# congliuUvA/Clifford-Group-Equivariant-Simplicial-Message-Passing-Networks

Hardware: AMD Instinct MI355X
Metric: simplicial edges/sec (fwd+bwd) on Cl(3,0) 8-ch multivectors; % HBM roofline (higher is better)
Workload: dtype f32; 1 GPU; S1: EGCL layer fwd+bwd, Cl(1, 1, 1), 8 channels, 10000 nodes, 100000 edges/GPU x 1 GPU, aggr=mean, edge_attr 6ch, node_attr 3ch; aggregation=float atomics, launch=hip-graph replay

## Files before the change

clifford-group-equivariant-simplicial-message-passing-networks_amd/csrc/cemlp_cl.hpp:

```cpp
#pragma once
#include "cemlp_lane.hpp"

namespace csmpn {

constexpr int kClWaves = 4;
constexpr int kClSliceCap = 512;
constexpr int kClParStride = 36;

#define CL_LDS_ORDER() do { asm volatile("" ::: "memory"); __builtin_amdgcn_wave_barrier(); asm volatile("" ::: "memory"); } while (0)

struct ClStamp {
#ifdef CSMPN_STAMPS
    static constexpr int kSlots = 24;
    unsigned long long t0, acc[kSlots];
    CSMPN_DEV explicit ClStamp(int) {
#pragma unroll
        for (int i = 0; i < kSlots; ++i) acc[i] = 0;
        t0 = __builtin_amdgcn_s_memtime();
    }
    CSMPN_DEV void operator()(int id) {
        __builtin_amdgcn_sched_barrier(0);
        const unsigned long long t1 = __builtin_amdgcn_s_memtime();
        acc[id] += t1 - t0;
        t0 = t1;
// ... 48 lines not shown
            "v_fmac_f32_dpp %0, %8, %16 row_ror:%20 row_mask:0xf bank_mask:0xf\n\t"
            "v_fmac_f32_dpp %1, %9, %17 row_ror:%20 row_mask:0xf bank_mask:0xf\n\t"
            "v_fmac_f32_dpp %2, %10, %17 row_ror:%20 row_mask:0xf bank_mask:0xf\n\t"
            "v_fmac_f32_dpp %3, %11, %17 row_ror:%20 row_mask:0xf bank_mask:0xf\n\t"
            "v_fmac_f32_dpp %4, %12, %18 row_ror:%20 row_mask:0xf bank_mask:0xf\n\t"
            "v_fmac_f32_dpp %5, %13, %18 row_ror:%20 row_mask:0xf bank_mask:0xf\n\t"
            "v_fmac_f32_dpp %6, %14, %18 row_ror:%20 row_mask:0xf bank_mask:0xf\n\t"
            "v_fmac_f32_dpp %7, %15, %19 row_ror:%20 row_mask:0xf bank_mask:0xf"
            : "+v"(acc[0]), "+v"(acc[1]), "+v"(acc[2]), "+v"(acc[3]), "+v"(acc[4]), "+v"(acc[5]), "+v"(acc[6]), "+v"(acc[7])
            : "v"(x[0]), "v"(x[1]), "v"(x[2]), "v"(x[3]), "v"(x[4]), "v"(x[5]), "v"(x[6]), "v"(x[7]),
              "v"(w.x), "v"(w.y), "v"(w.z), "v"(w.w), "n"(ROT));
    }
}

template <int NK>
CSMPN_DEV void cl_pin(f4 (&w)[NK]) {
    if constexpr (NK == 8) asm volatile("" : "+v"(w[0]), "+v"(w[1]), "+v"(w[2]), "+v"(w[3]), "+v"(w[4]), "+v"(w[5]), "+v"(w[6]), "+v"(w[7]));
    else if constexpr (NK == 4) asm volatile("" : "+v"(w[0]), "+v"(w[1]), "+v"(w[2]), "+v"(w[3]));
    else if constexpr (NK == 2) asm volatile("" : "+v"(w[0]), "+v"(w[1]));
    else static_assert(NK == 1 || NK == 2 || NK == 4 || NK == 8, "batch size");
}
template <int C, int NROT, int TOFF, int BATCH = 4>
CSMPN_DEV void cl_mix(float (&acc)[8], const float (&x)[8], const float* ldsw) {
    static_assert(NROT % BATCH == 0, "whole batches");
#ifdef CL_X_NOMIX
    cl_fmac8<0>(acc, x, ld4(ldsw + TOFF));
    return;
#endif
    constexpr int NB = NROT / BATCH;
    f4 w[BATCH];
#pragma unroll
    for (int i = 0; i < BATCH; ++i) w[i] = ld4(ldsw + (TOFF + 4 * C * i));
    cl_pin<BATCH>(w);
    static_for<0, NB>([&](auto b) {
        f4 wn[BATCH];
        if constexpr (b + 1 < NB) {
#pragma unroll
            for (int i = 0; i < BATCH; ++i) wn[i] = ld4(ldsw + (TOFF + 4 * C * (BATCH * (b + 1) + i)));
        }
        static_for<0, BATCH>([&](auto i) { cl_fmac8<ClMap<C>::ROTL * (BATCH * b + i)>(acc, x, w[i]); });
        if constexpr (b + 1 < NB) {
            cl_pin<BATCH>(wn);
#pragma unroll
            for (int i = 0; i < BATCH; ++i) w[i] = wn[i];
        }
    });
}

constexpr int cl_pow2_ge(int w) { int p = 1; while (p < w) p <<= 1; return p; }

template <int C, int MODE, int NA, int K, bool BWD>
struct ClTab {
    static constexpr int NSEG = MODE == MODE_EDGE ? 1 : (MODE == MODE_NODE ? 2 : 0);
    static_assert(MODE == MODE_EDGE || MODE == MODE_NODE, "edge or node program");
    static constexpr int NP = K > 0 ? 1 : NSEG + (NA > 0 ? 1 : 0);
    static constexpr int width(int p) { return (K > 0 || p < NSEG) ? C : NA; }
    static constexpr int period(int p) { return (K > 0 || p < NSEG) ? C : cl_pow2_ge(NA); }
    static constexpr int coff(int p) { return C * p; }
    static constexpr int I = K > 0 ? C : NSEG * C + NA;
    static_assert(NA <= C, "attribute segment wider than the layer");
    static constexpr int W1(int p) { int o = 0; for (int q = 0; q < p; ++q) o += 4 * C * period(q); return o; }
    static constexpr int WR = W1(NP), WL = WR + 4 * C * C;
    static constexpr int fwd_end = WL + 4 * C * C;
    static constexpr int W1T(int p) { return fwd_end + 4 * C * C * p; }
    static constexpr int WRT = W1T(NP), WLT = WRT + 4 * C * C;
    static constexpr int par = BWD ? WLT + 4 * C * C : fwd_end;
    static constexpr int total = par + C * kClParStride;
    static constexpr int n_entries = par / 4;
};

template <int C>
CSMPN_DEV size_t cl_state_off(long row, int c) {
    constexpr int RPT = 64 / C;
    return (size_t)(row / RPT) * 512 + 4 * ((int)(row % RPT) * C + c);
}
struct ClFwd {
    float y[8], gate[4], R[8], invden[4], s[8];
    float qs, nl, invMn;
};

CSMPN_DEV float cl_smooth_abs_sqrt(float q) { return sqrt_pos(sqrt_pos(__builtin_fmaf(q, q, kSmooth))); }

template <class ALG, int C, class TB, bool BWD>
__device__ void cl_stage_block(const DevBlock& B, float* base, int tid, int dir) {
    constexpr int G = ALG::G, P = ALG::P, NE = TB::n_entries, NIT = (NE + 64 * kClWaves - 1) / (64 * kClWaves);
    static_assert(G == 4, "the weight of one (o, c) pair is one 16-byte vector of 4 grades");
    const float *pW1 = B.W1, *pWR = B.WR, *pWL = B.WL;
    const float* src[NIT];
#pragma unroll
    for (int it = 0; it < NIT; ++it) {
        const int e = tid + it * 64 * kClWaves;
        src[it] = nullptr;
        static_for<0, TB::NP>([&](auto p) {
            constexpr int e0 = TB::W1(p) / 4, PER = TB::period(p), n = PER * C;
            if (e >= e0 && e < e0 + n) {
                const int k = (e - e0) / C, o = (e - e0) % C, cs = (o + dir * k) & (PER - 1);
                if (cs < TB::width(p)) src[it] = pW1 + ((o * TB::I + TB::coff(p) + cs) * G);
            }
        });
        if (e >= TB::WR / 4 && e < TB::fwd_end / 4) {
            const int f = e - TB::WR / 4, which = f / (C * C), k = (f % (C * C)) / C, o = f % C, cs = (o + dir * k) & (C - 1);
            src[it] = (which == 0 ? pWR : pWL) + ((o * C + cs) * G);
        }
        if constexpr (BWD) {
            static_for<0, TB::NP>([&](auto p) {
                constexpr int e0 = TB::W1T(p) / 4, PER = TB::period(p);
                if (e >= e0 && e < e0 + C * C) {
                    const int k = (e - e0) / C, c = (e - e0) % C, o = (c + dir * k) & (C - 1), cs = c & (PER - 1);
                    if (cs < TB::width(p)) src[it] = pW1 + ((o * TB::I + TB::coff(p) + cs) * G);
                }
            });
            if (e >= TB::WRT / 4 && e < TB::par / 4) {
                const int f = e - TB::WRT / 4, which = f / (C * C), k = (f % (C * C)) / C, c = f % C, o = (c + dir * k) & (C - 1);
                src[it] = (which == 0 ? pWR : pWL) + ((o * C + c) * G);
            }
        }
    }
    f4 v[NIT];
#pragma unroll
    for (int it = 0; it < NIT; ++it) v[it] = src[it] ? ld4(src[it]) : f4{0.f, 0.f, 0.f, 0.f};
    constexpr int NPAR = C * kClParStride, NITP = (NPAR + 64 * kClWaves - 1) / (64 * kClWaves);
    static_assert(16 + P <= kClParStride, "parameter stride");
    const float *pb1 = B.b1, *pbL = B.bL, *pla = B.la, *psa = B.sa, *psb = B.sb, *pan = B.an, *pw = B.w;
    const bool has_b1 = B.has_b1 != 0;
    const float* ps[NITP];
    bool sig[NITP];
#pragma unroll
    for (int it = 0; it < NITP; ++it) {
        const int e = tid + it * 64 * kClWaves;
        ps[it] = nullptr;
        sig[it] = false;
        if (e < NPAR) {
            const int ch = e / kClParStride, s = e % kClParStride;
            if (s == 0) { if (has_b1) ps[it] = pb1 + ch; }
            else if (s == 1) ps[it] = pbL + ch;
            else if (s == 2) ps[it] = pla + ch;
            else if (s >= 4 && s < 8) ps[it] = psa + ch * G + (s - 4);
            else if (s >= 8 && s < 12) ps[it] = psb + ch * G + (s - 8);
            else if (s >= 12 && s < 16) { ps[it] = pan + ch * G + (s - 12); sig[it] = true; }
            else if (s >= 16 && s < 16 + P) ps[it] = pw + ch * P + (s - 16);
        }
    }
    float pv[NITP];
#pragma unroll
    for (int it = 0; it < NITP; ++it) pv[it] = ps[it] ? *ps[it] : 0.f;
#pragma unroll
    for (int it = 0; it < NIT; ++it) {
        const int e = tid + it * 64 * kClWaves;
        if (e < NE) st4(base + 4 * e, v[it]);
    }
#pragma unroll
    for (int it = 0; it < NITP; ++it) {
        const int e = tid + it * 64 * kClWaves;
        if (sig[it]) pv[it] = sigmoidf(pv[it]);
        if (e < NPAR) base[TB::par + e] = pv[it];
    }
}

template <class ALG>
CSMPN_DEV void cl_weighted_gp(float (&out)[8], const float (&z)[8], const float (&r)[8], const float* wp) {
    constexpr int P = ALG::P;
    f4 wv[(P + 3) / 4];
#pragma unroll
    for (int q = 0; q < (P + 3) / 4; ++q) wv[q] = ld4(wp + 4 * q);
    static_for<0, P>([&](auto p) {
        constexpr int gi = ALG::t.path_g[p][0], gj = ALG::t.path_g[p][1], gk = ALG::t.path_g[p][2];
        constexpr int i0 = ALG::gstart(gi), ni = ALG::gsize(gi);
        constexpr int j0 = ALG::gstart(gj), nj = ALG::gsize(gj);
        constexpr int k0 = ALG::gstart(gk), nk = ALG::gsize(gk);
        const float w = wv[p / 4][p % 4];
        float tmp[nj];
#pragma unroll
        for (int t = 0; t < nj; ++t) tmp[t] = 0.f;
        static_for<0, ni>([&](auto ii) {
            static_for<0, nk>([&](auto kk) {
                constexpr int i = i0 + ii, k = k0 + kk;
                constexpr int j = ALG::t.out[i][k];
                if constexpr (j >= j0 && j < j0 + nj) {
                    constexpr float sg = float(ALG::t.sign[i][k]);
                    tmp[j - j0] += (sg * z[i]) * r[k];
                }
            });
        });
#pragma unroll
        for (int t = 0; t < nj; ++t) out[j0 + t] = __builtin_fmaf(w, tmp[t], out[j0 + t]);
    });
}

template <class ALG, int C, class TB, int BATCH>
CSMPN_DEV void cl_block_tail(const float* ldsw, const float* ldsp, ClFwd& S, float (&out)[8], ClStamp& stamp, int sid, bool have_s = false) {
    constexpr int D = ALG::D, G = ALG::G;
    static_assert(D == 8 && G == 4, "Cl(3,0)-shaped algebra");
    const f4 p0 = ld4(ldsp + TB::par);
    const f4 sa = ld4(ldsp + (TB::par + 4)), sb = ld4(ldsp + (TB::par + 8));
    S.y[0] += p0.x;
    float z[D];
    static_for<0, G>([&](auto g) {
        constexpr int d0 = ALG::gstart(g), nd = ALG::gsize(g);
        float u;
        if constexpr (g == 0) {
            u = S.y[0];
        } else {
            u = 0.f;
            static_for<0, nd>([&](auto t) {
                constexpr int d = d0 + decltype(t)::value;
                u += qsf<ALG, d> * S.y[d] * S.y[d];
            });
        }
        S.gate[g] = sigmoidf(__builtin_fmaf(sa[int(g)], u, sb[int(g)]));
#pragma unroll
        for (int t = 0; t < nd; ++t) z[d0 + t] = S.gate[g] * S.y[d0 + t];
    });
    stamp(sid);
    float L[D];
#pragma unroll
    for (int d = 0; d < D; ++d) { S.R[d] = 0.f; L[d] = 0.f; }
    cl_mix<C, C, TB::WR, BATCH>(S.R, z, ldsw);
    if (have_s) {
        const f4 sg = ld4(ldsp + (TB::par + 12));
        static_for<0, G>([&](auto g) {
            constexpr int d0 = ALG::gstart(g), nd = ALG::gsize(g);
            float qq = 0.f;
            static_for<0, nd>([&](auto t) {
                constexpr int d = d0 + decltype(t)::value;
                qq += qsf<ALG, d> * S.R[d] * S.R[d];
            });
            const float m = __builtin_fmaf(sg[int(g)], cl_smooth_abs_sqrt(qq) - 1.0f, 1.0f);
            S.invden[g] = fast_rcp(m + kEps);
        });
        float qs = 0.f;
        static_for<0, D>([&](auto dd) {
            constexpr int d = decltype(dd)::value;
            qs += qsf<ALG, d> * S.s[d] * S.s[d];
        });
        S.qs = qs;
        S.nl = cl_smooth_abs_sqrt(qs);
        S.invMn = fast_rcp(__builtin_fmaf(cl_chan_sum<C>(S.nl), 1.0f / float(C), kEps));
        return;
    }
    cl_mix<C, C, TB::WL, BATCH>(L, z, ldsw);
// ... 197 lines not shown
    stamp(sid + 5);
    const f4 sa = ld4(ldsp + (TB::par + 4));
    static_for<0, G>([&](auto g) {
        constexpr int d0 = ALG::gstart(g), nd = ALG::gsize(g);
        float ggate = 0.f;
#pragma unroll
        for (int t = 0; t < nd; ++t) ggate = __builtin_fmaf(gz[d0 + t], S.y[d0 + t], ggate);
        const float gpre = ggate * S.gate[g] * (1.0f - S.gate[g]);
        float u;
        if constexpr (g == 0) {
            u = S.y[0];
        } else {
            u = 0.f;
            static_for<0, nd>([&](auto t) {
                constexpr int d = d0 + decltype(t)::value;
                u += qsf<ALG, d> * S.y[d] * S.y[d];
            });
        }
        sm.template add<RM::i_sa + 2 * g>(gpre * u);
        sm.template add<RM::i_sa + 2 * g + 1>(gpre);
        const float gu = gpre * sa[int(g)];
        static_for<0, nd>([&](auto t) {
            constexpr int d = d0 + decltype(t)::value;
            float v = gz[d] * S.gate[g];
            if constexpr (g == 0) v += gu;
            else v = __builtin_fmaf(gu * (2.0f * qsf<ALG, d>), S.y[d], v);
            gy[d] = v;
        });
    });
    sm.template add<RM::i_b1>(gy[0]);
    stamp(sid + 6);
}

CSMPN_DEV void cl_ld8(float (&x)[8], const float* p) {
    const f4 a = ld4(p), b = ld4(p + 4);
    x[0] = a.x; x[1] = a.y; x[2] = a.z; x[3] = a.w; x[4] = b.x; x[5] = b.y; x[6] = b.z; x[7] = b.w;
}
CSMPN_DEV void cl_st8(float* p, const float (&x)[8]) {
    st4(p, f4{x[0], x[1], x[2], x[3]});
    st4(p + 4, f4{x[4], x[5], x[6], x[7]});
}
#ifdef CL_X_NOOUT
#define CL_GST8(gp, lp, x) cl_st8(lp, x)
#else
#define CL_GST8(gp, lp, x) cl_st8(gp, x)
#endif

template <int C, int ROWLEN, bool SUB>
CSMPN_DEV void cl_scatter(const float* sc, int t_add, int t_sub, float* table, int lane) {
    using MP = ClMap<C>;
    constexpr int RPW = MP::RPW, SS = ROWLEN + 4, NC = ROWLEN / 64;
    static_assert(ROWLEN % 64 == 0, "whole columns");
    static_for<0, NC>([&](auto cc) {
        const int colx = 64 * cc + lane;
        const float* col = sc + colx;
        auto flush = [&](int target, float a) {
#ifndef CL_X_NOOUT
            if (target >= 0) atomicAdd(table + (size_t)target * ROWLEN + colx, a);
#else
            if (target == -12345) atomicAdd(table + (size_t)target * ROWLEN + colx, a);
#endif
        };
        float val[RPW];
#pragma unroll
        for (int i = 0; i < RPW; ++i) val[i] = col[i * SS];
        float acc = 0.f;
        int cur = __builtin_amdgcn_readlane(t_add, MP::lane_of_row(0));
        static_for<0, RPW>([&](auto rr) {
            const int t = __builtin_amdgcn_readlane(t_add, MP::lane_of_row(rr));
            if (t != cur) {
                flush(cur, acc);
                cur = t;
                acc = 0.f;
            }
            acc += val[rr];
        });
        flush(cur, acc);
        if constexpr (SUB) {
            static_for<0, RPW>([&](auto rr) { flush(__builtin_amdgcn_readlane(t_sub, MP::lane_of_row(rr)), -val[rr]); });
        }
    });
}

template <int C, int MODE>
struct ClTile {
    long row, lrow;
    bool valid;
    int i_dst, i_src, i_perm;
    float scale;
    template <int NA>
    CSMPN_DEV void load(const RowIO& io, long tile, int r) {
        row = tile * ClMap<C>::RPW + r;
        valid = row < io.rows;
        lrow = valid ? row : 0;
        i_dst = i_src = i_perm = 0;
        scale = 1.0f;
        if constexpr (MODE == MODE_EDGE) {
            i_dst = io.seg[0].ia[lrow];
            i_src = io.seg[0].ib[lrow];
            if constexpr (NA > 0) i_perm = io.seg[1].ia[lrow];
        }
        if constexpr (MODE == MODE_NODE) {
            if (io.seg[1].deg) { const int dg = io.seg[1].deg[lrow]; scale = 1.0f / float(dg > 1 ? dg : 1); }
        }
    }
};

template <class ALG, int C, int MODE, int NA>
struct ClRaw {
    static constexpr int NSEG = MODE == MODE_EDGE ? 2 : 2;
    f4 v[2 * (NSEG + (NA > 0 ? 1 : 0))];
    template <class TB>
    CSMPN_DEV void issue(const RowIO& io, const ClTile<C, MODE>& T, int c) {
        constexpr int D = ALG::D, ROW = C * D;
        const float *p0, *p1, *p2 = nullptr;
        if constexpr (MODE == MODE_EDGE) {
            p0 = io.seg[0].a + (size_t)T.i_dst * ROW + c * D;
            p1 = io.seg[0].b + (size_t)T.i_src * ROW + c * D;
            if constexpr (NA > 0) {
                const int ca = c & (TB::period(1) - 1);
                p2 = io.seg[1].a + (size_t)T.i_perm * (NA * D) + (ca < NA ? ca : NA - 1) * D;
            }
        } else {
            p0 = io.seg[0].a + (size_t)T.lrow * ROW + c * D;
            p1 = io.seg[1].a + (size_t)T.lrow * ROW + c * D;
            if constexpr (NA > 0) {
                const int ca = c & (TB::period(2) - 1);
                p2 = io.seg[2].a + (size_t)T.lrow * (NA * D) + (ca < NA ? ca : NA - 1) * D;
            }
        }
        v[0] = ld4(p0); v[1] = ld4(p0 + 4);
        v[2] = ld4(p1); v[3] = ld4(p1 + 4);
        if constexpr (NA > 0) { v[4] = ld4(p2); v[5] = ld4(p2 + 4); }
    }
    CSMPN_DEV void pin() {
        if constexpr (NA > 0) asm volatile("" : "+v"(v[0]), "+v"(v[1]), "+v"(v[2]), "+v"(v[3]), "+v"(v[4]), "+v"(v[5]));
        else asm volatile("" : "+v"(v[0]), "+v"(v[1]), "+v"(v[2]), "+v"(v[3]));
    }
    template <class TB>
    CSMPN_DEV void finish(float (&x)[TB::NP][8], const ClTile<C, MODE>& T) const {
        auto unpack = [&](float (&t)[8], const f4& a, const f4& b) {
            t[0] = a.x; t[1] = a.y; t[2] = a.z; t[3] = a.w; t[4] = b.x; t[5] = b.y; t[6] = b.z; t[7] = b.w;
        };
        if constexpr (MODE == MODE_EDGE) {
            const f4 a = v[0] - v[2], b = v[1] - v[3];
            unpack(x[0], a, b);
            if constexpr (NA > 0) unpack(x[1], v[4], v[5]);
        } else {
            unpack(x[0], v[0], v[1]);
            unpack(x[1], v[2] * T.scale, v[3] * T.scale);
            if constexpr (NA > 0) unpack(x[2], v[4], v[5]);
        }
    }
};

template <int C>
CSMPN_DEV int cl_probe_dir(int c) {
    const int probe = cl_dpp_i<0x120 + ClMap<C>::ROTL>(c);
    return (((probe - c) & (C - 1)) == 1) ? 1 : -1;
}

template <class ALG, int C, int MODE, int NBLK, int NA>
__global__ void __launch_bounds__(64 * kClWaves, 4) cemlp_cl_fwd_kernel(const DevCemlp C_arg, const RowIO io_arg) {
    CSMPN_KERNEL_ARGS(Cd);
    using MP = ClMap<C>;
    using T0 = ClTab<C, MODE, NA, 0, false>;
    using T1 = ClTab<C, MODE, NA, 1, false>;
    constexpr int D = ALG::D, ROW = C * D, RPW = MP::RPW, SS = ROW + 4;
    static_assert(NBLK == 1 || NBLK == 2, "one or two blocks");
    constexpr int tab_floats = T0::total + (NBLK > 1 ? T1::total : 0);
    constexpr int kBatch = 4;
    extern __shared__ __attribute__((aligned(16))) float smem[];
    float* lds = smem;
    const int wave = threadIdx.x >> 6, lane = threadIdx.x & 63;
    const int c = MP::chan(lane), r = MP::row(lane);
    float* sc = lds + tab_floats + wave * (RPW * SS);
    ClStamp stamp(0);
    const float* ldsw0 = lds + 4 * c;
    const float* ldsp0 = lds + kClParStride * c;
    const float* ldsw1 = ldsw0 + T0::total;
    const float* ldsp1 = ldsp0 + T0::total;

    const long ntiles = (io.rows + RPW - 1) / RPW;
    const long tstride = (long)gridDim.x * kClWaves;
    const bool save_s = NBLK > 1 && io.save_state != 0 && io.save != nullptr;
    const long tile0 = (long)blockIdx.x * kClWaves + wave;
    ClTile<C, MODE> T, Tn;
    T.template load<NA>(io, tile0, r);
    ClRaw<ALG, C, MODE, NA> raw;
    raw.template issue<T0>(io, T, c);
    Tn.template load<NA>(io, tile0 + tstride, r);
    {
        const int dir = cl_probe_dir<C>(c);
        cl_stage_block<ALG, C, T0, false>(Cd.b[0], lds, threadIdx.x, dir);
        if constexpr (NBLK > 1) cl_stage_block<ALG, C, T1, false>(Cd.b[1], lds + T0::total, threadIdx.x, dir);
    }
    __syncthreads();
    stamp(0);
    for (long tile = tile0; tile < ntiles; tile += tstride) {
        raw.pin();
        stamp(1);
        float out[D], in1[D];
        {
            float x[T0::NP][D];
            raw.template finish<T0>(x, T);
            ClFwd S;
#pragma unroll
            for (int d = 0; d < D; ++d) S.y[d] = 0.f;
            static_for<0, T0::NP>([&](auto p) { cl_mix<C, T0::period(p), T0::W1(p), kBatch>(S.y, x[p], ldsw0); });
            stamp(2);
            cl_block_tail<ALG, C, T0, kBatch>(ldsw0, ldsp0, S, out, stamp, 3);
            if (save_s && T.valid) {
                float* ps_ = io.save + state_region<ROW, ROW>(io.rows, 0, 0) + cl_state_off<C>(T.row, c);
                __builtin_nontemporal_store(f4{S.s[0], S.s[1], S.s[2], S.s[3]}, reinterpret_cast<f4*>(ps_));
                __builtin_nontemporal_store(f4{S.s[4], S.s[5], S.s[6], S.s[7]}, reinterpret_cast<f4*>(ps_ + 256));
            }
        }
        if constexpr (NBLK > 1) {
#pragma unroll
            for (int d = 0; d < D; ++d) in1[d] = out[d];
            ClFwd S;
#pragma unroll
            for (int d = 0; d < D; ++d) S.y[d] = 0.f;
            cl_mix<C, C, T1::W1(0), kBatch>(S.y, in1, ldsw1);
            stamp(8);
            cl_block_tail<ALG, C, T1, kBatch>(ldsw1, ldsp1, S, out, stamp, 9);
            if (save_s && T.valid) {
                float* ps_ = io.save + state_region<ROW, ROW>(io.rows, 0, 1) + cl_state_off<C>(T.row, c);
                __builtin_nontemporal_store(f4{S.s[0], S.s[1], S.s[2], S.s[3]}, reinterpret_cast<f4*>(ps_));
                __builtin_nontemporal_store(f4{S.s[4], S.s[5], S.s[6], S.s[7]}, reinterpret_cast<f4*>(ps_ + 256));
            }
        }
        const ClTile<C, MODE> Tc = T;
        T = Tn;
        raw.template issue<T0>(io, T, c);
        Tn.template load<NA>(io, tile + 2 * tstride, r);
        if constexpr (NBLK > 1) {
            if (io.save && Tc.valid) CL_GST8(io.save + (size_t)Tc.row * ROW + c * D, sc + r * SS + c * D, in1);
        }
        if constexpr (MODE == MODE_EDGE) {
            if (io.row_store) {
                if (Tc.valid) CL_GST8(io.agg + (size_t)Tc.lrow * ROW + c * D, sc + r * SS + c * D, out);
            } else {
                CL_LDS_ORDER();
                cl_st8(sc + r * SS + c * D, out);
                CL_LDS_ORDER();
                cl_scatter<C, ROW, false>(sc, Tc.valid ? Tc.i_dst : -1, -1, io.agg, lane);
            }
        } else if (Tc.valid) {
            if (io.resid) {
                float res[D];
                cl_ld8(res, io.resid + (size_t)Tc.row * ROW + c * D);
#pragma unroll
                for (int d = 0; d < D; ++d) out[d] += res[d];
            }
            CL_GST8(io.y + (size_t)Tc.row * ROW + c * D, sc + r * SS + c * D, out);
        }
        stamp(14);
    }
    stamp.flush(io.stamps, lane);
}
template <class ALG, int C, int MODE, int NBLK, int NA>
constexpr size_t cl_fwd_lds_bytes() {
    return sizeof(float) * (ClTab<C, MODE, NA, 0, false>::total + (NBLK > 1 ? ClTab<C, MODE, NA, 1, false>::total : 0) +
                            (MODE == MODE_EDGE ? kClWaves * ClMap<C>::RPW * (C * ALG::D + 4) : 0));
}

struct ClCarry { f4 a, b; };
template <class ALG, int C, int MODE, int NBLK, int NA, int K, bool SAVES>
CSMPN_DEV ClCarry cl_bwd_block(const RowIO& io, float* tab, float* work, const ClCarry carry_in, bool single, ClStamp& stamp) {
    f4 carry_a = carry_in.a, carry_b = carry_in.b;
    using MP = ClMap<C>;
    using TB = ClTab<C, MODE, NA, K, true>;
    using PT = ClPart<ALG, C, TB::I>;
    using RM = ClRed<ALG>;
    constexpr int D = ALG::D, G = ALG::G, ROW = C * D, RPW = MP::RPW, SS = ROW + 4, NP = TB::NP;
    static_assert(K >= 0 && K < NBLK && NBLK <= 2, "block index");
    constexpr bool kLast = K == NBLK - 1;
    constexpr int img_max = NBLK > 1 && ClPart<ALG, C, C>::total > ClPart<ALG, C, ClTab<C, MODE, NA, 0, true>::I>::total
                                ? ClPart<ALG, C, C>::total : ClPart<ALG, C, ClTab<C, MODE, NA, 0, true>::I>::total;
    constexpr int scratch = (RPW * SS > img_max ? RPW * SS : img_max);
    const int wave = threadIdx.x >> 6, lane = threadIdx.x & 63;
    const int c = MP::chan(lane), r = MP::row(lane);
    float* sc = work + wave * scratch;
    const float* ldsw = tab + 4 * c;
    const float* ldsp = tab + kClParStride * c;

    f4 accW1[NP][G], accR[G], accL[G];
    ClSums<RM::n> sm(work + kClWaves * scratch + 4 * threadIdx.x);
    sm.zero();
#pragma unroll
    for (int g = 0; g < G; ++g) {
        accR[g] = accL[g] = f4{0.f, 0.f, 0.f, 0.f};
#pragma unroll
        for (int p = 0; p < NP; ++p) accW1[p][g] = f4{0.f, 0.f, 0.f, 0.f};
    }

    const long ntiles = (io.rows + RPW - 1) / RPW;
    const long tstride = (long)gridDim.x * kClWaves;
    f4 g0, g1, s0, s1;
    ClRaw<ALG, C, MODE, NA> raw;
    auto issue = [&](const ClTile<C, MODE>& Tl) {
        const float* gsrc = (kLast ? io.gy + (size_t)(MODE == MODE_EDGE ? (long)Tl.i_dst : Tl.lrow) * ROW
                                   : io.plw_g1 + (size_t)Tl.lrow * ROW) + c * D;
        if (kLast || !single) {
            g0 = ld4(gsrc); g1 = ld4(gsrc + 4);
        } else {
            g0 = carry_a; g1 = carry_b;
        }
        if constexpr (K == 0) {
            raw.template issue<TB>(io, Tl, c);
        } else {
            const float* sp = io.saved + (size_t)Tl.lrow * ROW + c * D;
            s0 = ld4(sp); s1 = ld4(sp + 4);
        }
    };
    const long tile0 = (long)blockIdx.x * kClWaves + wave;
    ClTile<C, MODE> T, Tn;
    T.template load<NA>(io, tile0, r);
    issue(T);
    Tn.template load<NA>(io, tile0 + tstride, r);
    for (long tile = tile0; tile < ntiles; tile += tstride) {
        if constexpr (K == 0) {
            asm volatile("" : "+v"(g0), "+v"(g1));
            raw.pin();
        } else {
            asm volatile("" : "+v"(g0), "+v"(g1), "+v"(s0), "+v"(s1));
        }
        stamp(1);
        const ClTile<C, MODE> Tc = T;
        float gout[D] = {g0.x, g0.y, g0.z, g0.w, g1.x, g1.y, g1.z, g1.w};
        float x[NP][D];
        if constexpr (K == 0) {
            raw.template finish<TB>(x, Tc);
        } else {
            x[0][0] = s0.x; x[0][1] = s0.y; x[0][2] = s0.z; x[0][3] = s0.w; x[0][4] = s1.x; x[0][5] = s1.y; x[0][6] = s1.z; x[0][7] = s1.w;
        }
        if (!Tc.valid) {
#pragma unroll
            for (int d = 0; d < D; ++d) gout[d] = 0.f;
        }
        float gy[D];
        {
            ClFwd S;
#pragma unroll
            for (int d = 0; d < D; ++d) S.y[d] = 0.f;
            constexpr bool have_s = SAVES;
            if constexpr (have_s) {
                const float* ps_ = io.saved + state_region<ROW, ROW>(io.rows, 0, K) + cl_state_off<C>(Tc.lrow, c);
                const f4 a_ = __builtin_nontemporal_load(reinterpret_cast<const f4*>(ps_)), b_ = __builtin_nontemporal_load(reinterpret_cast<const f4*>(ps_ + 256));
#pragma unroll
                for (int i = 0; i < 4; ++i) { S.s[i] = a_[i]; S.s[4 + i] = b_[i]; }
            }
            static_for<0, NP>([&](auto p) { cl_mix<C, TB::period(p), TB::W1(p)>(S.y, x[p], ldsw); });
            stamp(2);
            float unused[D];
            cl_block_tail<ALG, C, TB, 4>(ldsw, ldsp, S, unused, stamp, 3, have_s);
            cl_block_backward<ALG, C, TB>(ldsw, ldsp, S, gout, gy, sm, accR, accL, stamp, 8);
        }
#ifndef CL_X_NOMFMA
        static_for<0, NP>([&](auto p) {
            static_for<0, D>([&](auto d) { accW1[p][ALG::grade(d)] = mfma16(gy[d], x[p][d], accW1[p][ALG::grade(d)]); });
        });
#else
        static_for<0, NP>([&](auto p) { static_for<0, D>([&](auto d) { accW1[p][ALG::grade(d)][0] += gy[d] * x[p][d]; }); });
#endif
        stamp(15);
        T = Tn;
        issue(T);
        Tn.template load<NA>(io, tile + 2 * tstride, r);
        if constexpr (K > 0) {
            float gx[D];
#pragma unroll
            for (int d = 0; d < D; ++d) gx[d] = 0.f;
            cl_mix<C, C, TB::W1T(0)>(gx, gy, ldsw);
            if (single) {
                carry_a = f4{gx[0], gx[1], gx[2], gx[3]}; carry_b = f4{gx[4], gx[5], gx[6], gx[7]};
            } else if (Tc.valid) {
                CL_GST8(io.plw_g1 + (size_t)Tc.row * ROW + c * D, sc + r * SS + c * D, gx);
            }
        } else if constexpr (MODE == MODE_EDGE) {
            if (io.gx[0]) {
                float gx[D];
#pragma unroll
                for (int d = 0; d < D; ++d) gx[d] = 0.f;
                cl_mix<C, C, TB::W1T(0)>(gx, gy, ldsw);
                if (io.row_store) {
                    if (Tc.valid) CL_GST8(io.gx[0] + (size_t)Tc.lrow * ROW + c * D, sc + r * SS + c * D, gx);
                } else {
                    CL_LDS_ORDER();
                    cl_st8(sc + r * SS + c * D, gx);
                    CL_LDS_ORDER();
                    cl_scatter<C, ROW, true>(sc, Tc.valid ? Tc.i_dst : -1, Tc.valid ? Tc.i_src : -1, io.gx[0], lane);
                }
            }
            if constexpr (NA > 0) {
                if (io.gx[1]) {
                    float gx[D];
#pragma unroll
                    for (int d = 0; d < D; ++d) gx[d] = 0.f;
                    cl_mix<C, C, TB::W1T(1)>(gx, gy, ldsw);
                    if (Tc.valid && c < NA) CL_GST8(io.gx[1] + (size_t)Tc.i_perm * (NA * D) + c * D, sc + r * SS + c * D, gx);
                }
            }
        } else {
            if (io.gx[0]) {
                float gx[D];
#pragma unroll
                for (int d = 0; d < D; ++d) gx[d] = 0.f;
                cl_mix<C, C, TB::W1T(0)>(gx, gy, ldsw);
                if (Tc.valid) {
                    if (io.resid_bwd) {
                        float res[D];
                        cl_ld8(res, io.gy + (size_t)Tc.row * ROW + c * D);
#pragma unroll
                        for (int d = 0; d < D; ++d) gx[d] += res[d];
                    }
                    CL_GST8(io.gx[0] + (size_t)Tc.row * ROW + c * D, sc + r * SS + c * D, gx);
                }
            }
            if (io.gx[1]) {
                float gx[D];
#pragma unroll
                for (int d = 0; d < D; ++d) gx[d] = 0.f;
                cl_mix<C, C, TB::W1T(1)>(gx, gy, ldsw);
#pragma unroll
                for (int d = 0; d < D; ++d) gx[d] *= Tc.scale;
                if (Tc.valid) CL_GST8(io.gx[1] + (size_t)Tc.row * ROW + c * D, sc + r * SS + c * D, gx);
            }
            if constexpr (NA > 0) {
                if (io.gx[2]) {
                    float gx[D];
#pragma unroll
                    for (int d = 0; d < D; ++d) gx[d] = 0.f;
                    cl_mix<C, C, TB::W1T(2)>(gx, gy, ldsw);
                    if (Tc.valid && c < NA) CL_GST8(io.gx[2] + (size_t)Tc.row * (NA * D) + c * D, sc + r * SS + c * D, gx);
                }
            }
        }
        stamp(16);
    }

#ifdef CL_X_NOEND
    {
        f4 t = accR[0] + accL[0];
#pragma unroll
        for (int g = 0; g < G; ++g) { t += accR[g] + accL[g];
#pragma unroll
            for (int p = 0; p < NP; ++p) t += accW1[p][g]; }
        st4(sc + 4 * lane, t);
    }
    if (false)
#endif
    {
        float* img = sc;
        const int j = lane & 15, q = lane >> 4;
        auto put_tile = [&](const f4 (&acc)[G], int base, int I, int coff, int width) {
            if constexpr (C == 8) {
                float lo[G], hi[G];
#pragma unroll
                for (int g = 0; g < G; ++g) {
                    lo[g] = acc[g][0] + dpp_mov<0xB1>(acc[g][1]);
                    hi[g] = acc[g][2] + dpp_mov<0xB1>(acc[g][3]);
                }
                const int cc = j >> 1;
                if ((j & 1) == 0 && cc < width) {
                    float* p0 = img + base + ((2 * q) * I + coff + cc) * G;
                    st4(p0, f4{lo[0], lo[1], lo[2], lo[3]});
                    st4(p0 + I * G, f4{hi[0], hi[1], hi[2], hi[3]});
                }
            } else {
                if (j < width) {
#pragma unroll
                    for (int v = 0; v < 4; ++v) {
                        float* p0 = img + base + ((4 * q + v) * I + coff + j) * G;
                        st4(p0, f4{acc[0][v], acc[1][v], acc[2][v], acc[3][v]});
                    }
                }
            }
        };
        static_for<0, NP>([&](auto p) { put_tile(accW1[p], 0, TB::I, TB::coff(p), TB::width(p)); });
        put_tile(accR, PT::pWR, C, 0, C);
        put_tile(accL, PT::pWL, C, 0, C);
        f4 sv[ClSums<RM::n>::kGroups];
#pragma unroll
        for (int gq = 0; gq < ClSums<RM::n>::kGroups; ++gq) sv[gq] = ld4(sm.base + gq * (4 * 64 * kClWaves));
        static_for<0, RM::n>([&](auto idx) {
            const f4 t = __builtin_amdgcn_mfma_f32_16x16x4f32(1.0f, sv[idx / 4][idx % 4], f4{0.f, 0.f, 0.f, 0.f}, 0, 0, 0);
            float s = t[0];
            if constexpr (C == 8) s += dpp_mov<0xB1>(s);
            if (q == 0 && (C == 16 || (lane & 1) == 0)) img[PT::pS + PT::off(idx) + c * PT::stride(idx)] = s;
        });
        __syncthreads();
        float* part = io.rl_partials + (K == 0 ? 0 : (size_t)kClSliceCap * ClPart<ALG, C, ClTab<C, MODE, NA, 0, true>::I>::total) +
                      (size_t)blockIdx.x * PT::total;
        const float* img0 = work;
        static_assert(PT::total % 4 == 0, "slice length");
        for (int e = 4 * threadIdx.x; e < PT::total; e += 4 * 64 * kClWaves) {
            f4 v = ld4(img0 + e);
#pragma unroll
            for (int w = 1; w < kClWaves; ++w) v += ld4(img0 + w * scratch + e);
            st4(part + e, v);
        }
    }
    stamp(17);
    return ClCarry{carry_a, carry_b};
}
template <class ALG, int C, int MODE, int NBLK, int NA>
constexpr size_t cl_bwd_lds_bytes() {
    using TB0 = ClTab<C, MODE, NA, 0, true>;
    using TB1 = ClTab<C, MODE, NA, 1, true>;
    constexpr int tile = ClMap<C>::RPW * (C * ALG::D + 4);
    int img = ClPart<ALG, C, TB0::I>::total;
    if (NBLK > 1 && ClPart<ALG, C, C>::total > img) img = ClPart<ALG, C, C>::total;
    return sizeof(float) * (TB0::total + (NBLK > 1 ? TB1::total : 0) + kClWaves * (tile > img ? tile : img) +
                            ClSums<ClRed<ALG>::n>::floats_per_wg);
}
template <class ALG, int C, int MODE, int NBLK, int NA, bool SAVES = false>
__global__ void __launch_bounds__(64 * kClWaves, 2) cemlp_cl_bwd_kernel(const DevCemlp C_arg, const RowIO io_arg) {
    CSMPN_KERNEL_ARGS(Cd);
    extern __shared__ __attribute__((aligned(16))) float smem[];
    ClStamp stamp(0);
    using TB0 = ClTab<C, MODE, NA, 0, true>;
    using TB1 = ClTab<C, MODE, NA, 1, true>;
    constexpr int tabs = TB0::total + (NBLK > 1 ? TB1::total : 0);
    {
        const int dir = cl_probe_dir<C>(ClMap<C>::chan(threadIdx.x & 63));
        cl_stage_block<ALG, C, TB0, true>(Cd.b[0], smem, threadIdx.x, dir);
        if constexpr (NBLK > 1) cl_stage_block<ALG, C, TB1, true>(Cd.b[1], smem + TB0::total, threadIdx.x, dir);
    }
    __syncthreads();
    stamp(0);
    const long ntiles = (io.rows + ClMap<C>::RPW - 1) / ClMap<C>::RPW;
    const bool single = ntiles <= (long)gridDim.x * kClWaves;
    ClCarry carry{f4{0.f, 0.f, 0.f, 0.f}, f4{0.f, 0.f, 0.f, 0.f}};
    if constexpr (NBLK > 1) {
        carry = cl_bwd_block<ALG, C, MODE, NBLK, NA, 1, SAVES>(io, smem + TB0::total, smem + tabs, carry, single, stamp);
        asm volatile("s_waitcnt vmcnt(0)" ::: "memory");
        __syncthreads();
    }
    cl_bwd_block<ALG, C, MODE, NBLK, NA, 0, SAVES>(io, smem, smem + tabs, carry, single, stamp);
    stamp.flush(io.stamps, threadIdx.x & 63);
}

template <class ALG, int C, int I0, int NBLK>
__global__ void __launch_bounds__(256) cl_reduce_kernel(const DevCemlp Cd, const float* part, int nslices, int slice_cap) {
    constexpr int G = ALG::G;
    using P0 = ClPart<ALG, C, I0>;
    using P1 = ClPart<ALG, C, C>;
    constexpr int total = P0::total + (NBLK > 1 ? P1::total : 0);
    __shared__ float red[16][17];
    const int j = threadIdx.x & 15, w = threadIdx.x >> 4;
    int e = blockIdx.x * 16 + j;
    const bool live = e < total;
    if (!live) e = 0;
    const int k = (NBLK > 1 && e >= P0::total) ? 1 : 0;
    const int len = k == 0 ? P0::total : P1::total;
    const float* p = part + (k == 0 ? 0 : (size_t)slice_cap * P0::total);
    if (k == 1) e -= P0::total;
    float s = 0.f;
    for (int s0 = w; s0 < nslices; s0 += 256) {
        float v[16];
#pragma unroll
        for (int i = 0; i < 16; ++i) {
            const int sl = s0 + 16 * i;
            v[i] = sl < nslices ? p[(size_t)sl * len + e] : 0.f;
        }
#pragma unroll
        for (int i = 0; i < 16; ++i) s += v[i];
    }
    red[w][j] = s;
    __syncthreads();
    if (w != 0 || !live) return;
#pragma unroll
    for (int i = 1; i < 16; ++i) s += red[i][j];
    const DevBlock& B = Cd.b[k];
    const int I = k == 0 ? I0 : C;
    int f = e;
    float* dst = nullptr;
    const int nW1 = C * I * G, nWC = C * C * G;
    if (f < nW1) dst = B.gW1 + f;
    else if ((f -= nW1) < nWC) dst = B.gWR + f;
    else if ((f -= nWC) < nWC) dst = B.gWL + f;
    else {
        f -= nWC;
        if (f < P0::qsa) dst = B.has_b1 ? B.gb1 + f : nullptr;
        else if (f < P0::qsb) dst = B.gsa + (f - P0::qsa);
        else if (f < P0::qw) dst = B.gsb + (f - P0::qsb);
        else if (f < P0::qan) dst = B.gw + (f - P0::qw);
        else if (f < P0::qbL) dst = B.gan + (f - P0::qan);
        else if (f < P0::qla) dst = B.gbL + (f - P0::qbL);
        else dst = B.gla + (f - P0::qla);
    }
    if (dst) *dst += s;
}

}
```

Before: 566.8 million edges/s.

## Prefetch first-tile inputs before weight staging and specialize single-pass backward

The weight-staging routine becomes a struct that issues every global load before any LDS store, with branchless clamped addresses so loads can overlap. The backward kernel now requests the first tile's gradient, saved-activation and state loads before staging weights. It also compiles separate single-tile and multi-tile paths, and in the single-tile case issues the next block's loads before the reduction barrier. Residual loads in forward and backward are hoisted earlier and degree scaling is computed lazily. Together these hide global-memory latency behind LDS staging and barriers, at the cost of more live registers and code duplication from the template specialization.

```diff
diff --git a/clifford-group-equivariant-simplicial-message-passing-networks_amd/csrc/cemlp_cl.hpp b/clifford-group-equivariant-simplicial-message-passing-networks_amd/csrc/cemlp_cl.hpp
--- a/clifford-group-equivariant-simplicial-message-passing-networks_amd/csrc/cemlp_cl.hpp
+++ b/clifford-group-equivariant-simplicial-message-passing-networks_amd/csrc/cemlp_cl.hpp
@@ -154,80 +154,90 @@
 CSMPN_DEV float cl_smooth_abs_sqrt(float q) { return sqrt_pos(sqrt_pos(__builtin_fmaf(q, q, kSmooth))); }
 
 template <class ALG, int C, class TB, bool BWD>
-__device__ void cl_stage_block(const DevBlock& B, float* base, int tid, int dir) {
-    constexpr int G = ALG::G, P = ALG::P, NE = TB::n_entries, NIT = (NE + 64 * kClWaves - 1) / (64 * kClWaves);
+struct ClStage {
+    static constexpr int G = ALG::G, P = ALG::P, NE = TB::n_entries, NIT = (NE + 64 * kClWaves - 1) / (64 * kClWaves);
+    static constexpr int NPAR = C * kClParStride, NITP = (NPAR + 64 * kClWaves - 1) / (64 * kClWaves);
     static_assert(G == 4, "the weight of one (o, c) pair is one 16-byte vector of 4 grades");
-    const float *pW1 = B.W1, *pWR = B.WR, *pWL = B.WL;
-    const float* src[NIT];
-#pragma unroll
-    for (int it = 0; it < NIT; ++it) {
-        const int e = tid + it * 64 * kClWaves;
-        src[it] = nullptr;
-        static_for<0, TB::NP>([&](auto p) {
-            constexpr int e0 = TB::W1(p) / 4, PER = TB::period(p), n = PER * C;
-            if (e >= e0 && e < e0 + n) {
-                const int k = (e - e0) / C, o = (e - e0) % C, cs = (o + dir * k) & (PER - 1);
-                if (cs < TB::width(p)) src[it] = pW1 + ((o * TB::I + TB::coff(p) + cs) * G);
-            }
-        });
-        if (e >= TB::WR / 4 && e < TB::fwd_end / 4) {
-            const int f = e - TB::WR / 4, which = f / (C * C), k = (f % (C * C)) / C, o = f % C, cs = (o + dir * k) & (C - 1);
-            src[it] = (which == 0 ? pWR : pWL) + ((o * C + cs) * G);
-        }
-        if constexpr (BWD) {
+    static_assert(16 + P <= kClParStride, "parameter stride");
+    f4 v[NIT];
+    float pv[NITP];
+    bool live[NIT], plive[NITP], sig[NITP];
+    __device__ void load(const DevBlock& B, int tid, int dir) {
+        const float *pW1 = B.W1, *pWR = B.WR, *pWL = B.WL;
+        const float* src[NIT];
+#pragma unroll
+        for (int it = 0; it < NIT; ++it) {
+            const int e = tid + it * 64 * kClWaves;
+            src[it] = nullptr;
             static_for<0, TB::NP>([&](auto p) {
-                constexpr int e0 = TB::W1T(p) / 4, PER = TB::period(p);
-                if (e >= e0 && e < e0 + C * C) {
-                    const int k = (e - e0) / C, c = (e - e0) % C, o = (c + dir * k) & (C - 1), cs = c & (PER - 1);
+                constexpr int e0 = TB::W1(p) / 4, PER = TB::period(p), n = PER * C;
+                if (e >= e0 && e < e0 + n) {
+                    const int k = (e - e0) / C, o = (e - e0) % C, cs = (o + dir * k) & (PER - 1);
                     if (cs < TB::width(p)) src[it] = pW1 + ((o * TB::I + TB::coff(p) + cs) * G);
                 }
             });
-            if (e >= TB::WRT / 4 && e < TB::par / 4) {
-                const int f = e - TB::WRT / 4, which = f / (C * C), k = (f % (C * C)) / C, c = f % C, o = (c + dir * k) & (C - 1);
-                src[it] = (which == 0 ? pWR : pWL) + ((o * C + c) * G);
-            }
-        }
-    }
-    f4 v[NIT];
-#pragma unroll
-    for (int it = 0; it < NIT; ++it) v[it] = src[it] ? ld4(src[it]) : f4{0.f, 0.f, 0.f, 0.f};
-    constexpr int NPAR = C * kClParStride, NITP = (NPAR + 64 * kClWaves - 1) / (64 * kClWaves);
-    static_assert(16 + P <= kClParStride, "parameter stride");
-    const float *pb1 = B.b1, *pbL = B.bL, *pla = B.la, *psa = B.sa, *psb = B.sb, *pan = B.an, *pw = B.w;
-    const bool has_b1 = B.has_b1 != 0;
-    const float* ps[NITP];
-    bool sig[NITP];
-#pragma unroll
-    for (int it = 0; it < NITP; ++it) {
-        const int e = tid + it * 64 * kClWaves;
-        ps[it] = nullptr;
-        sig[it] = false;
-        if (e < NPAR) {
-            const int ch = e / kClParStride, s = e % kClParStride;
-            if (s == 0) { if (has_b1) ps[it] = pb1 + ch; }
-            else if (s == 1) ps[it] = pbL + ch;
-            else if (s == 2) ps[it] = pla + ch;
-            else if (s >= 4 && s < 8) ps[it] = psa + ch * G + (s - 4);
-            else if (s >= 8 && s < 12) ps[it] = psb + ch * G + (s - 8);
-            else if (s >= 12 && s < 16) { ps[it] = pan + ch * G + (s - 12); sig[it] = true; }
-            else if (s >= 16 && s < 16 + P) ps[it] = pw + ch * P + (s - 16);
-        }
-    }
-    float pv[NITP];
-#pragma unroll
-    for (int it = 0; it < NITP; ++it) pv[it] = ps[it] ? *ps[it] : 0.f;
-#pragma unroll
-    for (int it = 0; it < NIT; ++it) {
-        const int e = tid + it * 64 * kClWaves;
-        if (e < NE) st4(base + 4 * e, v[it]);
-    }
-#pragma unroll
-    for (int it = 0; it < NITP; ++it) {
-        const int e = tid + it * 64 * kClWaves;
-        if (sig[it]) pv[it] = sigmoidf(pv[it]);
-        if (e < NPAR) base[TB::par + e] = pv[it];
-    }
-}
+            if (e >= TB::WR / 4 && e < TB::fwd_end / 4) {
+                const int f = e - TB::WR / 4, which = f / (C * C), k = (f % (C * C)) / C, o = f % C, cs = (o + dir * k) & (C - 1);
+                src[it] = (which == 0 ? pWR : pWL) + ((o * C + cs) * G);
+            }
+            if constexpr (BWD) {
+                static_for<0, TB::NP>([&](auto p) {
+                    constexpr int e0 = TB::W1T(p) / 4, PER = TB::period(p);
+                    if (e >= e0 && e < e0 + C * C) {
+                        const int k = (e - e0) / C, c = (e - e0) % C, o = (c + dir * k) & (C - 1), cs = c & (PER - 1);
+                        if (cs < TB::width(p)) src[it] = pW1 + ((o * TB::I + TB::coff(p) + cs) * G);
+                    }
+                });
+                if (e >= TB::WRT / 4 && e < TB::par / 4) {
+                    const int f = e - TB::WRT / 4, which = f / (C * C), k = (f % (C * C)) / C, c = f % C, o = (c + dir * k) & (C - 1);
+                    src[it] = (which == 0 ? pWR : pWL) + ((o * C + c) * G);
+                }
+            }
+        }
+#pragma unroll
+        for (int it = 0; it < NIT; ++it) {
+            live[it] = src[it] != nullptr;
+            v[it] = ld4(live[it] ? src[it] : pW1);
+        }
+        const float *pb1 = B.b1, *pbL = B.bL, *pla = B.la, *psa = B.sa, *psb = B.sb, *pan = B.an, *pw = B.w;
+        const bool has_b1 = B.has_b1 != 0;
+        const float* ps[NITP];
+#pragma unroll
+        for (int it = 0; it < NITP; ++it) {
+            const int e = tid + it * 64 * kClWaves;
+            ps[it] = nullptr;
+            sig[it] = false;
+            if (e < NPAR) {
+                const int ch = e / kClParStride, s = e % kClParStride;
+                if (s == 0) { if (has_b1) ps[it] = pb1 + ch; }
+                else if (s == 1) ps[it] = pbL + ch;
+                else if (s == 2) ps[it] = pla + ch;
+                else if (s >= 4 && s < 8) ps[it] = psa + ch * G + (s - 4);
+                else if (s >= 8 && s < 12) ps[it] = psb + ch * G + (s - 8);
+                else if (s >= 12 && s < 16) { ps[it] = pan + ch * G + (s - 12); sig[it] = true; }
+                else if (s >= 16 && s < 16 + P) ps[it] = pw + ch * P + (s - 16);
+            }
+        }
+#pragma unroll
+        for (int it = 0; it < NITP; ++it) {
+            plive[it] = ps[it] != nullptr;
+            pv[it] = *(plive[it] ? ps[it] : pW1);
+        }
+    }
+    __device__ void store(float* base, int tid) {
+#pragma unroll
+        for (int it = 0; it < NIT; ++it) {
+            const int e = tid + it * 64 * kClWaves;
+            if (e < NE) st4(base + 4 * e, live[it] ? v[it] : f4{0.f, 0.f, 0.f, 0.f});
+        }
+#pragma unroll
+        for (int it = 0; it < NITP; ++it) {
+            const int e = tid + it * 64 * kClWaves;
+            if (sig[it]) pv[it] = sigmoidf(pv[it]);
+            if (e < NPAR) base[TB::par + e] = plive[it] ? pv[it] : 0.f;
+        }
+    }
+};
 
 template <class ALG>
 CSMPN_DEV void cl_weighted_gp(float (&out)[8], const float (&z)[8], const float (&r)[8], const float* wp) {
@@ -591,26 +601,27 @@
     });
 }
 
+__device__ const int kClNoDegree = 1;
 template <int C, int MODE>
 struct ClTile {
     long row, lrow;
     bool valid;
-    int i_dst, i_src, i_perm;
-    float scale;
+    int i_dst, i_src, i_perm, deg;
+    CSMPN_DEV float scale() const { return 1.0f / float(deg > 1 ? deg : 1); }
     template <int NA>
     CSMPN_DEV void load(const RowIO& io, long tile, int r) {
         row = tile * ClMap<C>::RPW + r;
         valid = row < io.rows;
         lrow = valid ? row : 0;
         i_dst = i_src = i_perm = 0;
-        scale = 1.0f;
+        deg = 1;
         if constexpr (MODE == MODE_EDGE) {
             i_dst = io.seg[0].ia[lrow];
             i_src = io.seg[0].ib[lrow];
             if constexpr (NA > 0) i_perm = io.seg[1].ia[lrow];
         }
         if constexpr (MODE == MODE_NODE) {
-            if (io.seg[1].deg) { const int dg = io.seg[1].deg[lrow]; scale = 1.0f / float(dg > 1 ? dg : 1); }
+            deg = *(io.seg[1].deg ? io.seg[1].deg + lrow : &kClNoDegree);
         }
     }
 };
@@ -657,7 +668,8 @@
             if constexpr (NA > 0) unpack(x[1], v[4], v[5]);
         } else {
             unpack(x[0], v[0], v[1]);
-            unpack(x[1], v[2] * T.scale, v[3] * T.scale);
+            const float sc_ = T.scale();
+            unpack(x[1], v[2] * sc_, v[3] * sc_);
             if constexpr (NA > 0) unpack(x[2], v[4], v[5]);
         }
     }
@@ -701,14 +713,25 @@
     Tn.template load<NA>(io, tile0 + tstride, r);
     {
         const int dir = cl_probe_dir<C>(c);
-        cl_stage_block<ALG, C, T0, false>(Cd.b[0], lds, threadIdx.x, dir);
-        if constexpr (NBLK > 1) cl_stage_block<ALG, C, T1, false>(Cd.b[1], lds + T0::total, threadIdx.x, dir);
+        ClStage<ALG, C, T0, false> st0;
+        ClStage<ALG, C, T1, false> st1;
+        st0.load(Cd.b[0], threadIdx.x, dir);
+        if constexpr (NBLK > 1) st1.load(Cd.b[1], threadIdx.x, dir);
+        st0.store(lds, threadIdx.x);
+        if constexpr (NBLK > 1) st1.store(lds + T0::total, threadIdx.x);
     }
     __syncthreads();
     stamp(0);
     for (long tile = tile0; tile < ntiles; tile += tstride) {
         raw.pin();
         stamp(1);
+        f4 res0, res1;
+        if constexpr (MODE == MODE_NODE) {
+            if (io.resid) {
+                const float* pr_ = io.resid + (size_t)T.lrow * ROW + c * D;
+                res0 = ld4(pr_); res1 = ld4(pr_ + 4);
+            }
+        }
         float out[D], in1[D];
         {
             float x[T0::NP][D];
@@ -758,8 +781,7 @@
             }
         } else if (Tc.valid) {
             if (io.resid) {
-                float res[D];
-                cl_ld8(res, io.resid + (size_t)Tc.row * ROW + c * D);
+                const float res[D] = {res0.x, res0.y, res0.z, res0.w, res1.x, res1.y, res1.z, res1.w};
 #pragma unroll
                 for (int d = 0; d < D; ++d) out[d] += res[d];
             }
@@ -776,8 +798,39 @@
 }
 
 struct ClCarry { f4 a, b; };
-template <class ALG, int C, int MODE, int NBLK, int NA, int K, bool SAVES>
-CSMPN_DEV ClCarry cl_bwd_block(const RowIO& io, float* tab, float* work, const ClCarry carry_in, bool single, ClStamp& stamp) {
+template <class ALG, int C, int MODE, int NBLK, int NA, bool SAVES>
+struct ClBwdReq {
+    f4 g0, g1, s0, s1, t0, t1;
+    ClRaw<ALG, C, MODE, NA> raw;
+    template <int K>
+    CSMPN_DEV void request(const RowIO& io, const ClTile<C, MODE>& Tl, int c) {
+        constexpr int D = ALG::D, ROW = C * D;
+        if constexpr (K == NBLK - 1) {
+            const float* gsrc = io.gy + (size_t)(MODE == MODE_EDGE ? (long)Tl.i_dst : Tl.lrow) * ROW + c * D;
+            g0 = ld4(gsrc); g1 = ld4(gsrc + 4);
+        }
+        if constexpr (K == 0) {
+            raw.template issue<ClTab<C, MODE, NA, 0, true>>(io, Tl, c);
+        } else {
+            const float* sp = io.saved + (size_t)Tl.lrow * ROW + c * D;
+            s0 = ld4(sp); s1 = ld4(sp + 4);
+        }
+        if constexpr (SAVES) {
+            const float* ps_ = io.saved + state_region<ROW, ROW>(io.rows, 0, K) + cl_state_off<C>(Tl.lrow, c);
+            t0 = __builtin_nontemporal_load(reinterpret_cast<const f4*>(ps_));
+            t1 = __builtin_nontemporal_load(reinterpret_cast<const f4*>(ps_ + 256));
+        }
+    }
+    CSMPN_DEV void arrived0() {
+        raw.pin();
+        if constexpr (SAVES) asm volatile("" : "+v"(t0), "+v"(t1));
+    }
+};
+template <class ALG, int C, int MODE, int NBLK, int NA, int K, bool SAVES, bool SINGLE>
+CSMPN_DEV ClCarry cl_bwd_block(const RowIO& io, float* tab, float* work, const ClTile<C, MODE>& T0,
+                               ClBwdReq<ALG, C, MODE, NBLK, NA, SAVES>& cur,
+                               ClBwdReq<ALG, C, MODE, NBLK, NA, SAVES>& next, const ClCarry carry_in, ClStamp& stamp) {
+    constexpr bool single = SINGLE, have_pre = SINGLE || K == NBLK - 1;
     f4 carry_a = carry_in.a, carry_b = carry_in.b;
     using MP = ClMap<C>;
     using TB = ClTab<C, MODE, NA, K, true>;
@@ -807,12 +860,12 @@
 
     const long ntiles = (io.rows + RPW - 1) / RPW;
     const long tstride = (long)gridDim.x * kClWaves;
-    f4 g0, g1, s0, s1;
-    ClRaw<ALG, C, MODE, NA> raw;
+    f4 &g0 = cur.g0, &g1 = cur.g1, &s0 = cur.s0, &s1 = cur.s1, &t0 = cur.t0, &t1 = cur.t1;
+    ClRaw<ALG, C, MODE, NA>& raw = cur.raw;
     auto issue = [&](const ClTile<C, MODE>& Tl) {
         const float* gsrc = (kLast ? io.gy + (size_t)(MODE == MODE_EDGE ? (long)Tl.i_dst : Tl.lrow) * ROW
                                    : io.plw_g1 + (size_t)Tl.lrow * ROW) + c * D;
-        if (kLast || !single) {
+        if constexpr (kLast || !single) {
             g0 = ld4(gsrc); g1 = ld4(gsrc + 4);
         } else {
             g0 = carry_a; g1 = carry_b;
@@ -825,10 +878,14 @@
         }
     };
     const long tile0 = (long)blockIdx.x * kClWaves + wave;
-    ClTile<C, MODE> T, Tn;
-    T.template load<NA>(io, tile0, r);
-    issue(T);
-    Tn.template load<NA>(io, tile0 + tstride, r);
+    ClTile<C, MODE> T = T0, Tn = T0;
+    if constexpr (have_pre) {
+        if constexpr (!kLast) { g0 = carry_a; g1 = carry_b; }
+    } else {
+        issue(T);
+    }
+    if constexpr (!single) Tn.template load<NA>(io, tile0 + tstride, r);
+    stamp(20);
     for (long tile = tile0; tile < ntiles; tile += tstride) {
         if constexpr (K == 0) {
             asm volatile("" : "+v"(g0), "+v"(g1));
@@ -856,16 +913,26 @@
             for (int d = 0; d < D; ++d) S.y[d] = 0.f;
             constexpr bool have_s = SAVES;
             if constexpr (have_s) {
-                const float* ps_ = io.saved + state_region<ROW, ROW>(io.rows, 0, K) + cl_state_off<C>(Tc.lrow, c);
-                const f4 a_ = __builtin_nontemporal_load(reinterpret_cast<const f4*>(ps_)), b_ = __builtin_nontemporal_load(reinterpret_cast<const f4*>(ps_ + 256));
-#pragma unroll
-                for (int i = 0; i < 4; ++i) { S.s[i] = a_[i]; S.s[4 + i] = b_[i]; }
+                if (!have_pre || (!single && tile != tile0)) {
+                    const float* ps_ = io.saved + state_region<ROW, ROW>(io.rows, 0, K) + cl_state_off<C>(Tc.lrow, c);
+                    t0 = __builtin_nontemporal_load(reinterpret_cast<const f4*>(ps_));
+                    t1 = __builtin_nontemporal_load(reinterpret_cast<const f4*>(ps_ + 256));
+                }
+#pragma unroll
+                for (int i = 0; i < 4; ++i) { S.s[i] = t0[i]; S.s[4 + i] = t1[i]; }
             }
             static_for<0, NP>([&](auto p) { cl_mix<C, TB::period(p), TB::W1(p)>(S.y, x[p], ldsw); });
             stamp(2);
             float unused[D];
             cl_block_tail<ALG, C, TB, 4>(ldsw, ldsp, S, unused, stamp, 3, have_s);
             cl_block_backward<ALG, C, TB>(ldsw, ldsp, S, gout, gy, sm, accR, accL, stamp, 8);
+        }
+        f4 res0, res1;
+        if constexpr (K == 0 && MODE == MODE_NODE && single) {
+            if (io.gx[0] && io.resid_bwd) {
+                const float* pr_ = io.gy + (size_t)Tc.lrow * ROW + c * D;
+                res0 = ld4(pr_); res1 = ld4(pr_ + 4);
+            }
         }
 #ifndef CL_X_NOMFMA
         static_for<0, NP>([&](auto p) {
@@ -875,15 +942,17 @@
         static_for<0, NP>([&](auto p) { static_for<0, D>([&](auto d) { accW1[p][ALG::grade(d)][0] += gy[d] * x[p][d]; }); });
 #endif
         stamp(15);
-        T = Tn;
-        issue(T);
-        Tn.template load<NA>(io, tile + 2 * tstride, r);
+        if constexpr (!single) {
+            T = Tn;
+            issue(T);
+            Tn.template load<NA>(io, tile + 2 * tstride, r);
+        }
         if constexpr (K > 0) {
             float gx[D];
 #pragma unroll
             for (int d = 0; d < D; ++d) gx[d] = 0.f;
             cl_mix<C, C, TB::W1T(0)>(gx, gy, ldsw);
-            if (single) {
+            if constexpr (single) {
                 carry_a = f4{gx[0], gx[1], gx[2], gx[3]}; carry_b = f4{gx[4], gx[5], gx[6], gx[7]};
             } else if (Tc.valid) {
                 CL_GST8(io.plw_g1 + (size_t)Tc.row * ROW + c * D, sc + r * SS + c * D, gx);
@@ -920,8 +989,11 @@
                 cl_mix<C, C, TB::W1T(0)>(gx, gy, ldsw);
                 if (Tc.valid) {
                     if (io.resid_bwd) {
-                        float res[D];
-                        cl_ld8(res, io.gy + (size_t)Tc.row * ROW + c * D);
+                        if constexpr (!single) {
+                            const float* pr_ = io.gy + (size_t)Tc.row * ROW + c * D;
+                            res0 = ld4(pr_); res1 = ld4(pr_ + 4);
+                        }
+                        const float res[D] = {res0.x, res0.y, res0.z, res0.w, res1.x, res1.y, res1.z, res1.w};
 #pragma unroll
                         for (int d = 0; d < D; ++d) gx[d] += res[d];
                     }
@@ -934,7 +1006,7 @@
                 for (int d = 0; d < D; ++d) gx[d] = 0.f;
                 cl_mix<C, C, TB::W1T(1)>(gx, gy, ldsw);
 #pragma unroll
-                for (int d = 0; d < D; ++d) gx[d] *= Tc.scale;
+                for (int d = 0; d < D; ++d) gx[d] *= Tc.scale();
                 if (Tc.valid) CL_GST8(io.gx[1] + (size_t)Tc.row * ROW + c * D, sc + r * SS + c * D, gx);
             }
             if constexpr (NA > 0) {
@@ -948,7 +1020,9 @@
             }
         }
         stamp(16);
-    }
+        if constexpr (single) break;
+    }
+    if constexpr (K > 0 && single) next.template request<K - 1>(io, T0, c);
 
 #ifdef CL_X_NOEND
     {
@@ -1000,7 +1074,10 @@
             if constexpr (C == 8) s += dpp_mov<0xB1>(s);
             if (q == 0 && (C == 16 || (lane & 1) == 0)) img[PT::pS + PT::off(idx) + c * PT::stride(idx)] = s;
         });
+        stamp(21);
         __syncthreads();
+        stamp(22);
+        if constexpr (K == 1 && single) next.arrived0();
         float* part = io.rl_partials + (K == 0 ? 0 : (size_t)kClSliceCap * ClPart<ALG, C, ClTab<C, MODE, NA, 0, true>::I>::total) +
                       (size_t)blockIdx.x * PT::total;
         const float* img0 = work;
@@ -1025,6 +1102,25 @@
     return sizeof(float) * (TB0::total + (NBLK > 1 ? TB1::total : 0) + kClWaves * (tile > img ? tile : img) +
                             ClSums<ClRed<ALG>::n>::floats_per_wg);
 }
+template <class ALG, int C, int MODE, int NBLK, int NA, bool SAVES, bool SINGLE>
+CSMPN_DEV void cl_bwd_blocks(const RowIO& io, float* smem, const ClTile<C, MODE>& T0, ClBwdReq<ALG, C, MODE, NBLK, NA, SAVES>& req,
+                             ClStamp& stamp) {
+    using TB0 = ClTab<C, MODE, NA, 0, true>;
+    using TB1 = ClTab<C, MODE, NA, 1, true>;
+    constexpr int tabs = TB0::total + (NBLK > 1 ? TB1::total : 0);
+    ClCarry carry{f4{0.f, 0.f, 0.f, 0.f}, f4{0.f, 0.f, 0.f, 0.f}};
+    if constexpr (NBLK > 1) {
+        ClBwdReq<ALG, C, MODE, NBLK, NA, SAVES> req0;
+        carry = cl_bwd_block<ALG, C, MODE, NBLK, NA, 1, SAVES, SINGLE>(io, smem + TB0::total, smem + tabs, T0, req, req0, carry, stamp);
+        if constexpr (!SINGLE) asm volatile("s_waitcnt vmcnt(0)" ::: "memory");
+        stamp(18);
+        __syncthreads();
+        stamp(19);
+        cl_bwd_block<ALG, C, MODE, NBLK, NA, 0, SAVES, SINGLE>(io, smem, smem + tabs, T0, req0, req, carry, stamp);
+    } else {
+        cl_bwd_block<ALG, C, MODE, NBLK, NA, 0, SAVES, SINGLE>(io, smem, smem + tabs, T0, req, req, carry, stamp);
+    }
+}
 template <class ALG, int C, int MODE, int NBLK, int NA, bool SAVES = false>
 __global__ void __launch_bounds__(64 * kClWaves, 2) cemlp_cl_bwd_kernel(const DevCemlp C_arg, const RowIO io_arg) {
     CSMPN_KERNEL_ARGS(Cd);
@@ -1033,22 +1129,27 @@
     using TB0 = ClTab<C, MODE, NA, 0, true>;
     using TB1 = ClTab<C, MODE, NA, 1, true>;
     constexpr int tabs = TB0::total + (NBLK > 1 ? TB1::total : 0);
+    ClTile<C, MODE> T0;
+    ClBwdReq<ALG, C, MODE, NBLK, NA, SAVES> req;
+    {
+        const int lane = threadIdx.x & 63;
+        T0.template load<NA>(io, (long)blockIdx.x * kClWaves + (threadIdx.x >> 6), ClMap<C>::row(lane));
+        req.template request<NBLK - 1>(io, T0, ClMap<C>::chan(lane));
+    }
     {
         const int dir = cl_probe_dir<C>(ClMap<C>::chan(threadIdx.x & 63));
-        cl_stage_block<ALG, C, TB0, true>(Cd.b[0], smem, threadIdx.x, dir);
-        if constexpr (NBLK > 1) cl_stage_block<ALG, C, TB1, true>(Cd.b[1], smem + TB0::total, threadIdx.x, dir);
+        ClStage<ALG, C, TB0, true> st0;
+        ClStage<ALG, C, TB1, true> st1;
+        st0.load(Cd.b[0], threadIdx.x, dir);
+        if constexpr (NBLK > 1) st1.load(Cd.b[1], threadIdx.x, dir);
+        st0.store(smem, threadIdx.x);
+        if constexpr (NBLK > 1) st1.store(smem + TB0::total, threadIdx.x);
     }
     __syncthreads();
     stamp(0);
     const long ntiles = (io.rows + ClMap<C>::RPW - 1) / ClMap<C>::RPW;
-    const bool single = ntiles <= (long)gridDim.x * kClWaves;
-    ClCarry carry{f4{0.f, 0.f, 0.f, 0.f}, f4{0.f, 0.f, 0.f, 0.f}};
-    if constexpr (NBLK > 1) {
-        carry = cl_bwd_block<ALG, C, MODE, NBLK, NA, 1, SAVES>(io, smem + TB0::total, smem + tabs, carry, single, stamp);
-        asm volatile("s_waitcnt vmcnt(0)" ::: "memory");
-        __syncthreads();
-    }
-    cl_bwd_block<ALG, C, MODE, NBLK, NA, 0, SAVES>(io, smem, smem + tabs, carry, single, stamp);
+    if (ntiles <= (long)gridDim.x * kClWaves) cl_bwd_blocks<ALG, C, MODE, NBLK, NA, SAVES, true>(io, smem, T0, req, stamp);
+    else cl_bwd_blocks<ALG, C, MODE, NBLK, NA, SAVES, false>(io, smem, T0, req, stamp);
     stamp.flush(io.stamps, threadIdx.x & 63);
 }
 
```

New measurement: 579.9 million edges/s (median of 6 runs). +2.3%, better.
